# arielgabizon/barretenberg

Hardware: AMD Instinct MI355X
Metric: BN254 G1 MSM points/sec at n=2^20 (Fr NTT elems/sec in 'ntt') (higher is better)
Workload: dtype u32x9 (256-bit Montgomery, 29-bit limbs)

## Files before the change

### barretenberg_amd/csrc/msm.hip

```cpp
#include <hip/hip_runtime.h>

#include <algorithm>
#include <mutex>
#include <stdint.h>
#include <stdio.h>
#include <stdlib.h>
#include <string.h>
#include <vector>

#include "bbgpu_internal.h"
#include "g1.hpp"
#include "g1_quad.hpp"
#include "host_g1.hpp"

namespace bbgpu {

using Fr = FrP;
#define FRONT_PRIO() __builtin_amdgcn_s_setprio(2)
constexpr int TAIL_PRIO = 3;
constexpr int SCALAR_BITS = 254;
constexpr int MSM_MAX_C = 16;
constexpr int MSM_THREADS = 256;

__device__ __forceinline__ void ld8(const uint32_t* p, uint32_t (&w)[8])
{
    const uint4* q = reinterpret_cast<const uint4*>(p);
    uint4 a = q[0], b = q[1];
    w[0] = a.x; w[1] = a.y; w[2] = a.z; w[3] = a.w;
    w[4] = b.x; w[5] = b.y; w[6] = b.z; w[7] = b.w;
}
__device__ __forceinline__ void ld16(const uint32_t* p, uint32_t (&w)[16])
{
    const uint4* q = reinterpret_cast<const uint4*>(p);
#pragma unroll
    for (int i = 0; i < 4; i++) {
        uint4 a = q[i];
        w[4 * i] = a.x; w[4 * i + 1] = a.y; w[4 * i + 2] = a.z; w[4 * i + 3] = a.w;
    }
}
__device__ __forceinline__ void st32(uint32_t* p, const uint32_t (&w)[32])
{
    uint4* q = reinterpret_cast<uint4*>(p);
#pragma unroll
    for (int i = 0; i < 8; i++) q[i] = make_uint4(w[4 * i], w[4 * i + 1], w[4 * i + 2], w[4 * i + 3]);
}
__device__ __forceinline__ void ld32(const uint32_t* p, uint32_t (&w)[32])
{
    const uint4* q = reinterpret_cast<const uint4*>(p);
#pragma unroll
    for (int i = 0; i < 8; i++) {
        uint4 a = q[i];
        w[4 * i] = a.x; w[4 * i + 1] = a.y; w[4 * i + 2] = a.z; w[4 * i + 3] = a.w;
    }
}

struct WinLayout {
    uint16_t off[66];
};
static WinLayout make_layout(int c, bool balanced)
{
    WinLayout LO{};
    const int W = msm_num_windows(c);
    if (!balanced) {
        for (int w = 0; w <= W; w++) LO.off[w] = (uint16_t)(c * w);
        return LO;
    }
    const int base = SCALAR_BITS / W, rem = SCALAR_BITS - base * W;
    int bit = 0;
    for (int w = 0; w < W; w++) {
        LO.off[w] = (uint16_t)bit;
        bit += base + (w < rem ? 1 : 0);
    }
    LO.off[W] = (uint16_t)bit;
    return LO;
}
__global__ void srs_convert_kernel(const uint32_t* __restrict__ table, uint32_t* __restrict__ srs, uint32_t n, uint32_t stride_words)
{
    const uint32_t i = blockIdx.x * blockDim.x + threadIdx.x;
    if (i >= n) return;
    uint32_t w[16];
    ld16(table + (size_t)i * stride_words, w);
    AffineV<2> a;
    load_affine_m256(a, w);
    uint32_t o[16];
    store_affine_m261(o, a.x, a.y);
    uint4* q = reinterpret_cast<uint4*>(srs + (size_t)i * 16);
#pragma unroll
    for (int k = 0; k < 4; k++) q[k] = make_uint4(o[4 * k], o[4 * k + 1], o[4 * k + 2], o[4 * k + 3]);
}

__global__ void srs_export_kernel(const uint32_t* __restrict__ srs, uint32_t* __restrict__ table, uint32_t n)
{
    const uint32_t i = blockIdx.x * blockDim.x + threadIdx.x;
    if (i >= n) return;
    uint32_t w[16];
    ld16(srs + (size_t)i * 16, w);
// ... 78 lines not shown
    return pow_u256<Fq>(a, e);
}
__global__ void srs_gen_points_kernel(const uint32_t* __restrict__ tab, Limbs9 x261, uint32_t* __restrict__ srs, uint32_t n, uint32_t first)
{
    const uint32_t i = blockIdx.x * blockDim.x + threadIdx.x;
    if (i >= n) return;
    Fe<Fr, 1, 2> s = fe_one<Fr>(), b = fe_from<Fr>(x261.d);
    for (uint32_t e = first + i; e; e >>= 1) {
        if (e & 1) s = mul(s, b);
        b = sqr(b);
    }
    uint32_t k[8];
    {
        FeT<Fr> one_raw = fe_zero<Fr>();
        one_raw.d[0] = 1;
        to_canonical(mul(s, one_raw), k);
    }
    Xyzz acc;
    set_infinity(acc);
    for (uint32_t w = 0; w < 32; w++) {
        const uint32_t d = (k[w >> 2] >> ((w & 3) * 8)) & 0xff;
        if (d) {
            uint32_t pw[32];
            ld32(tab + ((size_t)w * 256 + d) * 32, pw);
            Xyzz q;
            load_xyzz(q, pw);
            Xyzz t;
            add(t, acc, q);
            acc = t;
        }
    }
    auto inv = fq_inverse(mul(acc.zz, acc.zzz));
    auto izz = mul(inv, acc.zzz), izzz = mul(inv, acc.zz);
    uint32_t o[16];
    store_affine_m261(o, mul(acc.x, izz), mul(acc.y, izzz));
    uint4* q = reinterpret_cast<uint4*>(srs + (size_t)i * 16);
#pragma unroll
    for (int t = 0; t < 4; t++) q[t] = make_uint4(o[4 * t], o[4 * t + 1], o[4 * t + 2], o[4 * t + 3]);
}

struct ScalarSets {
    const uint32_t* p[MSM_MAX_JOBS];
};
template <class DT> struct DigitTraits { static constexpr bool wide = false; };
template <> struct DigitTraits<uint16_t> { static constexpr bool wide = true; };
template <class DT> __device__ __forceinline__ int load_digit(const DT* __restrict__ dg, const unsigned long long* __restrict__ sg, uint32_t i)
{
    if constexpr (DigitTraits<DT>::wide) {
        const int u = dg[i];
        return ((sg[i >> 6] >> (i & 63u)) & 1ull) ? -u - 1 : u;
    } else {
        return dg[i];
    }
}
template <class DT> __device__ __forceinline__ void load_digits8(const DT* __restrict__ dg, const unsigned long long* __restrict__ sg, uint32_t i8, int (&d)[8])
{
    const uint4 q = *reinterpret_cast<const uint4*>(dg + i8);
    const uint32_t w[4] = { q.x, q.y, q.z, q.w };
    if constexpr (DigitTraits<DT>::wide) {
        const uint32_t sb = reinterpret_cast<const uint8_t*>(sg)[i8 >> 3];
#pragma unroll
        for (int k = 0; k < 8; k++) {
            const int u = (int)((w[k >> 1] >> (16 * (k & 1))) & 0xffffu);
            d[k] = ((sb >> k) & 1u) ? -u - 1 : u;
        }
    } else {
#pragma unroll
        for (int k = 0; k < 8; k++) d[k] = (int)(int16_t)(w[k >> 1] >> (16 * (k & 1)));
    }
}
template <class DT> __global__ void __launch_bounds__(MSM_THREADS) msm_digits_kernel(ScalarSets sets, DT* __restrict__ digits_all, unsigned long long* __restrict__ signs_all,
                                                               uint32_t n, WinLayout LO, uint32_t num_windows, uint32_t wb, uint32_t we)
{
    FRONT_PRIO();
    const uint32_t i = blockIdx.x * blockDim.x + threadIdx.x;
    if (i >= n) return;
    const uint32_t* __restrict__ scalars = sets.p[blockIdx.y];
    DT* __restrict__ digits = digits_all + (size_t)blockIdx.y * num_windows * n;
    const uint32_t s64 = (n + 63) >> 6;
    unsigned long long* __restrict__ signs = signs_all + (size_t)blockIdx.y * num_windows * s64;
    uint32_t w[8], k[9];
    ld8(scalars + (size_t)i * 8, w);
    to_canonical(exact_limbs(mul(unpack<Fr>(w), fe_from<Fr>(Fr::M256_TO_PLAIN))), w);
#pragma unroll
    for (int j = 0; j < 8; j++) k[j] = w[j];
    k[8] = 0;
    uint32_t carry = 0;
    for (uint32_t win = 0; win < we; win++) {
        const uint32_t bit = LO.off[win], sz = LO.off[win + 1] - bit, j = bit >> 5, s = bit & 31;
        const uint32_t half = 1u << (sz - 1), mask = (1u << sz) - 1;
        uint32_t v = 0;
        if (j < 8) {
            v = k[j] >> s;
            if (s + sz > 32) v |= k[j + 1] << (32 - s);
        }
        v = (v & mask) + carry;
        carry = (win + 1 < num_windows && v >= half) ? 1u : 0u;
        const int32_t d = (int32_t)v - (int32_t)(carry << sz);
        if (win >= wb) {
            if constexpr (DigitTraits<DT>::wide) {
                const unsigned long long neg = __ballot(d < 0);
                digits[(size_t)win * n + i] = (DT)(d < 0 ? -d - 1 : d);
                if ((threadIdx.x & 63u) == 0) signs[(size_t)win * s64 + (i >> 6)] = neg;
            } else {
                digits[(size_t)win * n + i] = (DT)d;
            }
        }
    }
}

constexpr int SORT_THREADS = 1024;
constexpr uint32_t SORT_MAX_LB = 7;
constexpr uint32_t SORTB_MAX_PARTS = 8;
constexpr uint32_t SORTB_SPLIT_MIN = 1u << 16;

__device__ __forceinline__ bool wave_keys_heavy(bool valid, uint32_t key)
{
    const uint64_t vm = __ballot(valid);
    if (!vm) return false;
    const uint32_t k0 = __builtin_amdgcn_readlane(key, __ffsll((unsigned long long)vm) - 1);
    return 4 * __popcll(__ballot(valid && key == k0)) >= __popcll(vm);
}
__device__ __forceinline__ uint32_t lds_inc_dedup(uint32_t* ctr, uint32_t key, bool heavy)
{
    if (!heavy) return atomicAdd(&ctr[key], 1u);
    const uint32_t lane = __lane_id();
    uint64_t todo = __ballot(1);
    uint32_t res = 0;
    for (int it = 0; it < 4 && todo; it++) {
        const int leader = __ffsll((unsigned long long)todo) - 1;
        const uint32_t kk = __builtin_amdgcn_readlane(key, leader);
        const uint64_t m = __ballot(key == kk) & todo;
        uint32_t base = 0;
        if ((int)lane == leader) base = atomicAdd(&ctr[kk], (uint32_t)__popcll(m));
        base = __builtin_amdgcn_readlane(base, leader);
        if ((m >> lane) & 1ull) res = base + (uint32_t)__popcll(m & ((1ull << lane) - 1ull));
        todo &= ~m;
    }
    if ((todo >> lane) & 1ull) res = atomicAdd(&ctr[key], 1u);
    return res;
}

template <class DT> __global__ void __launch_bounds__(SORT_THREADS) __attribute__((amdgpu_num_vgpr(32))) sortA_hist_kernel(const DT* __restrict__ digits, const unsigned long long* __restrict__ signs, uint32_t* __restrict__ histA, uint32_t n,
                                                                uint32_t bins, uint32_t lb, uint32_t slices, uint32_t slice_len, uint32_t win0,
                                                                uint32_t wpg, uint32_t first_i0, uint32_t last_i1, uint32_t blo, uint32_t bcnt)
{
    FRONT_PRIO();
    __shared__ uint32_t lh[SORT_THREADS];
    const uint32_t s = blockIdx.x, wl = blockIdx.y;
    lh[threadIdx.x] = 0;
    __syncthreads();
    const uint32_t lo = s * slice_len, hi = min(n, lo + slice_len);
    const uint32_t s64 = (n + 63) >> 6;
    if ((n & 7u) == 0) {
        const uint32_t lo8 = lo & ~7u, bpw = lo < hi ? (((hi + 7u) & ~7u) - lo8) >> 3 : 0u;
        for (uint32_t u = threadIdx.x; u < wpg * bpw; u += SORT_THREADS) {
            const uint32_t k = u / bpw, i8 = lo8 + (u - k * bpw) * 8;
            const uint32_t klo = (k == 0) ? max(lo, first_i0) : lo, khi = (k + 1 == wpg) ? min(hi, last_i1) : hi;
            int d[8];
            load_digits8<DT>(digits + (size_t)(win0 + wl * wpg + k) * n, signs + (size_t)(win0 + wl * wpg + k) * s64, i8, d);
            const bool heavy = wave_keys_heavy(d[0] != 0, (uint32_t)((d[0] < 0 ? -d[0] : d[0]) - 1) >> lb);
#pragma unroll
            for (int j = 0; j < 8; j++)
                if (d[j] && i8 + j >= klo && i8 + j < khi) {
                    const uint32_t b = (uint32_t)((d[j] < 0 ? -d[j] : d[j]) - 1);
                    if (b - blo < bcnt) (void)lds_inc_dedup(lh, b >> lb, heavy);
                }
        }
    } else {
        for (uint32_t k = 0; k < wpg; k++) {
            const DT* dg = digits + (size_t)(win0 + wl * wpg + k) * n;
            const unsigned long long* sg = signs + (size_t)(win0 + wl * wpg + k) * s64;
            const uint32_t klo = (k == 0) ? max(lo, first_i0) : lo, khi = (k + 1 == wpg) ? min(hi, last_i1) : hi;
            for (uint32_t i = klo + threadIdx.x; i < khi; i += SORT_THREADS) {
                const int d = load_digit<DT>(dg, sg, i);
                if (d) {
                    const uint32_t b = (uint32_t)((d < 0 ? -d : d) - 1);
                    if (b - blo < bcnt) atomicAdd(&lh[b >> lb], 1u);
                }
            }
        }
// ... 342 lines not shown
            if (base + k * THREADS + t < end) buf[toff[(v[k] >> 24) & 0x7f] + rk[k]] = v[k];
        __syncthreads();
        const uint32_t tile_n = min(TILE, end - base);
        for (uint32_t x = t; x < tile_n; x += THREADS) {
            const uint32_t w = buf[x];
            sorted[dlt[(w >> 24) & 0x7f] + x] = w & 0x80ffffffu;
        }
    }
}

__device__ __forceinline__ void store_raw(uint32_t* dst, const Xyzz& p)
{
#if defined(__HIP_DEVICE_COMPILE__)
    uint32_t v[4 * NL];
#pragma unroll
    for (int i = 0; i < NL; i++) { v[i] = p.x.d[i]; v[NL + i] = p.y.d[i]; v[2 * NL + i] = p.zz.d[i]; v[3 * NL + i] = p.zzz.d[i]; }
#pragma unroll
    for (int i = 0; i < 4 * NL; i += 2)
        asm volatile("global_store_dwordx2 %0, %1, off offset:%2" :: "v"(dst), "v"(((unsigned long long)v[i + 1] << 32) | v[i]), "n"(4 * i) : "memory");
#else
#pragma unroll
    for (int i = 0; i < NL; i++) {
        dst[i] = p.x.d[i];
        dst[NL + i] = p.y.d[i];
        dst[2 * NL + i] = p.zz.d[i];
        dst[3 * NL + i] = p.zzz.d[i];
    }
#endif
}
__device__ __forceinline__ void load_raw(Xyzz& p, const uint32_t* src)
{
#pragma unroll
    for (int i = 0; i < NL; i++) {
        p.x.d[i] = src[i];
        p.y.d[i] = src[NL + i];
        p.zz.d[i] = src[2 * NL + i];
        p.zzz.d[i] = src[3 * NL + i];
    }
}
typedef uint32_t u32x4 __attribute__((ext_vector_type(4)));
struct RowRegs { u32x4 q0, q1, q2, q3; };
__device__ __forceinline__ void row_request(RowRegs& r, const uint32_t* p)
{
#if defined(__HIP_DEVICE_COMPILE__)
    asm volatile("global_load_dwordx4 %0, %4, off\n\t"
                 "global_load_dwordx4 %1, %4, off offset:16\n\t"
                 "global_load_dwordx4 %2, %4, off offset:32\n\t"
                 "global_load_dwordx4 %3, %4, off offset:48"
                 : "=&v"(r.q0), "=&v"(r.q1), "=&v"(r.q2), "=&v"(r.q3) : "v"(p) : "memory");
#else
    const u32x4* q = reinterpret_cast<const u32x4*>(p);
    r.q0 = q[0]; r.q1 = q[1]; r.q2 = q[2]; r.q3 = q[3];
#endif
}
__device__ __forceinline__ void row_land(RowRegs& r, uint32_t (&w)[16])
{
#if defined(__HIP_DEVICE_COMPILE__)
    __builtin_amdgcn_s_waitcnt(0x0f70);
    asm volatile("" : "+v"(r.q0), "+v"(r.q1), "+v"(r.q2), "+v"(r.q3));
#endif
#pragma unroll
    for (int i = 0; i < 4; i++) { w[i] = r.q0[i]; w[4 + i] = r.q1[i]; w[8 + i] = r.q2[i]; w[12 + i] = r.q3[i]; }
}
__device__ __forceinline__ void value_landed(uint32_t& v)
{
#if defined(__HIP_DEVICE_COMPILE__)
    asm volatile("" : "+v"(v));
#endif
}
__device__ __forceinline__ void operand_done(Fe<Fq, 1, 1>& x, Fe<Fq, 1, 2>& y)
{
#if defined(__HIP_DEVICE_COMPILE__)
    asm volatile("" : "+v"(x.d[0]), "+v"(x.d[1]), "+v"(x.d[2]), "+v"(x.d[3]), "+v"(x.d[4]), "+v"(x.d[5]), "+v"(x.d[6]), "+v"(x.d[7]), "+v"(x.d[8]));
    asm volatile("" : "+v"(y.d[0]), "+v"(y.d[1]), "+v"(y.d[2]), "+v"(y.d[3]), "+v"(y.d[4]), "+v"(y.d[5]), "+v"(y.d[6]), "+v"(y.d[7]), "+v"(y.d[8]));
#endif
}
constexpr int RAW_WORDS = 4 * NL;
constexpr uint32_t HEAVY_WGS = 256;
constexpr uint32_t HEAVY_IDS = 1 + HEAVY_WGS;
static_assert(MSM_THREADS == (int)HEAVY_WGS, "heavy-bucket queue header is cleared / combined by one lane per K4h workgroup");

__global__ void __launch_bounds__(MSM_THREADS) msm_accumulate_kernel(const uint32_t* __restrict__ srs, const uint32_t* __restrict__ sorted,
                                                                   const uint32_t* __restrict__ gstart, uint32_t* __restrict__ partials,
                                                                   uint32_t total_buckets, uint32_t ch, uint32_t prio, uint32_t* __restrict__ heavy_counter)
{
    if (heavy_counter && blockIdx.x == 0) {
        heavy_counter[threadIdx.x] = 0;
        if (threadIdx.x == 0) heavy_counter[MSM_THREADS] = 0;
    }
    if (prio == 1) __builtin_amdgcn_s_setprio(1);
    else if (prio == 2) __builtin_amdgcn_s_setprio(2);
    const uint32_t t = blockIdx.x * blockDim.x + threadIdx.x;
    const uint32_t M = gstart[total_buckets];
    const uint32_t p0 = t * ch;
    if (p0 >= M) return;
    const uint32_t p1 = min(M, p0 + ch);
    uint32_t lo = 0, hi = total_buckets;
    while (hi - lo > 1) {
        const uint32_t mid = (lo + hi) >> 1;
        if (gstart[mid] <= p0) lo = mid; else hi = mid;
    }
    uint32_t b = lo;
    uint32_t next_end = gstart[b + 1];
    Xyzz acc;
    set_infinity(acc);
    uint32_t after_next = gstart[min(b + 2, total_buckets + 1)];
    bool acc_inf = true;
    uint32_t v = sorted[p0];
    uint32_t vn = sorted[p0 + 1 < p1 ? p0 + 1 : p0];
    RowRegs row;
    uint32_t w[16];
    row_request(row, srs + (size_t)(v & 0x7fffffffu) * 16);
    Fe<Fq, 1, 1> px;
    Fe<Fq, 1, 2> py;
    row_land(row, w);
    load_affine_m261_signed(px, py, w, (v >> 31) != 0);
    operand_done(px, py);
    row_request(row, srs + (size_t)(vn & 0x7fffffffu) * 16);
    uint32_t e = p0;
    uint32_t trips = ch;
    do {
        const uint32_t vnn = sorted[min(e + 2, p1 - 1)];
        const bool start = (e == next_end) || acc_inf;
        if (start) {
            if (e == next_end) {
                store_raw(partials + (size_t)(b + t) * RAW_WORDS, acc);
                b++;
                next_end = after_next;
                if (next_end <= e) {
                    if (e >= M) {
                        b = total_buckets;
                    } else {
                        uint32_t l2 = b, h2 = total_buckets;
                        while (h2 - l2 > 1) {
                            const uint32_t mid = (l2 + h2) >> 1;
                            if (gstart[mid] <= e) l2 = mid; else h2 = mid;
                        }
                        b = l2;
                    }
                    next_end = gstart[b + 1];
                    value_landed(next_end);
                }
                after_next = gstart[min(b + 2, total_buckets + 1)];
            }
            acc.x = px;
            acc.y = py;
            acc.zz = fe_one<Fq>();
            acc.zzz = fe_one<Fq>();
            acc_inf = false;
        }
        asm volatile("" ::: "memory");
        if (!start) madd_ip(acc, acc_inf, px, py);
        row_land(row, w);
        load_affine_m261_signed(px, py, w, (vn >> 31) != 0);
        operand_done(px, py);
        row_request(row, srs + (size_t)(vnn & 0x7fffffffu) * 16);
        vn = vnn;
        e++;
    } while (--trips != 0);
    store_raw(partials + (size_t)(b + t) * RAW_WORDS, acc);
}

__device__ __forceinline__ Xyzz shfl_down_xyzz(const Xyzz& p, uint32_t off)
{
    Xyzz r;
#pragma unroll
    for (int i = 0; i < NL; i++) {
        r.x.d[i] = __shfl_down(p.x.d[i], off);
        r.y.d[i] = __shfl_down(p.y.d[i], off);
        r.zz.d[i] = __shfl_down(p.zz.d[i], off);
        r.zzz.d[i] = __shfl_down(p.zzz.d[i], off);
    }
    return r;
}
#define TAIL_OCC __attribute__((amdgpu_waves_per_eu(4, 4)))
constexpr int FOLD_T = 256;
constexpr int FOLD_LDS_WORDS = (FOLD_T / 2) * RAW_WORDS;
__device__ __forceinline__ void wg_tree_sum(Xyzz& acc, uint32_t* sh, uint32_t T, uint32_t t)
{
    constexpr uint32_t STRIDE = FOLD_T / 2;
    for (uint32_t half = T >> 1; half >= 1; half >>= 1) {
        if (t >= half && t < 2 * half) {
#pragma unroll
            for (int i = 0; i < NL; i++) {
                sh[(0 * NL + i) * STRIDE + t - half] = acc.x.d[i];
                sh[(1 * NL + i) * STRIDE + t - half] = acc.y.d[i];
                sh[(2 * NL + i) * STRIDE + t - half] = acc.zz.d[i];
                sh[(3 * NL + i) * STRIDE + t - half] = acc.zzz.d[i];
            }
        }
        __syncthreads();
        if (t < half) {
            Xyzz q, r;
#pragma unroll
            for (int i = 0; i < NL; i++) {
                q.x.d[i] = sh[(0 * NL + i) * STRIDE + t];
                q.y.d[i] = sh[(1 * NL + i) * STRIDE + t];
                q.zz.d[i] = sh[(2 * NL + i) * STRIDE + t];
                q.zzz.d[i] = sh[(3 * NL + i) * STRIDE + t];
            }
            add(r, acc, q);
            acc = r;
        }
        __syncthreads();
    }
}
__global__ void __launch_bounds__(MSM_THREADS) TAIL_OCC msm_merge_kernel(const uint32_t* __restrict__ gstart, const uint32_t* __restrict__ partials,
                                                              uint32_t* __restrict__ buckets, uint32_t* __restrict__ heavy, uint32_t bucket_begin, uint32_t total_buckets,
                                                              uint32_t ch, uint32_t MERGE_LIGHT, uint32_t logG)
{
    __builtin_amdgcn_s_setprio(TAIL_PRIO);
    const uint32_t t = blockIdx.x * blockDim.x + threadIdx.x;
    const uint32_t G = 1u << logG, b = bucket_begin + (t >> logG), j = t & (G - 1);
    if (b >= total_buckets) return;
    const uint32_t s = gstart[b], e = gstart[b + 1];
    Xyzz acc;
    set_infinity(acc);
    if (e > s) {
        const uint32_t t0 = s / ch, t1 = (e - 1) / ch;
        if (t1 - t0 >= MERGE_LIGHT) {
            if (j == 0) heavy[HEAVY_IDS + atomicAdd(&heavy[0], 1u)] = b;
            return;
        }
        for (uint32_t k = t0 + j; k <= t1; k += G) {
            Xyzz q, r;
            load_raw(q, partials + (size_t)(b + k) * RAW_WORDS);
            add(r, acc, q);
            acc = r;
        }
    }
    for (uint32_t off = G >> 1; off >= 1; off >>= 1) {
        const Xyzz o = shfl_down_xyzz(acc, off);
        if (j < off) {
            Xyzz r;
            add(r, acc, o);
            acc = r;
        }
    }
    if (j == 0) {
        uint32_t o[32];
        store_xyzz(o, acc);
        st32(buckets + (size_t)b * 32, o);
    }
}
__global__ void __launch_bounds__(MSM_THREADS) TAIL_OCC msm_merge_heavy_kernel(const uint32_t* __restrict__ gstart, const uint32_t* __restrict__ partials,
                                                                    uint32_t* __restrict__ buckets, uint32_t* __restrict__ heavy, uint32_t ch, uint32_t* __restrict__ hpart)
{
    __builtin_amdgcn_s_setprio(TAIL_PRIO);
    __shared__ uint32_t sh[FOLD_LDS_WORDS];
    __shared__ uint32_t last_flag;
    const uint32_t count = heavy[0];
    const uint32_t K = count ? gridDim.x / count : 0;
    if (K < 2) {
        for (uint32_t item = blockIdx.x; item < count; item += gridDim.x) {
            const uint32_t b = heavy[HEAVY_IDS + item];
            const uint32_t s = gstart[b], e = gstart[b + 1];
            const uint32_t t0 = s / ch, t1 = (e - 1) / ch;
            Xyzz acc;
            set_infinity(acc);
            for (uint32_t t = t0 + threadIdx.x; t <= t1; t += MSM_THREADS) {
                Xyzz q, r;
                load_raw(q, partials + (size_t)(b + t) * RAW_WORDS);
                add(r, acc, q);
                acc = r;
            }
            __syncthreads();
            wg_tree_sum(acc, sh, MSM_THREADS, threadIdx.x);
            if (threadIdx.x == 0) {
                uint32_t o[32];
                store_xyzz(o, acc);
                st32(buckets + (size_t)b * 32, o);
            }
        }
        return;
    }
    const uint32_t item = blockIdx.x / K, sub = blockIdx.x - item * K;
    if (item >= count) return;
    const uint32_t b = heavy[HEAVY_IDS + item];
    const uint32_t s = gstart[b], e = gstart[b + 1];
    const uint32_t t0 = s / ch, t1 = (e - 1) / ch, total = t1 - t0 + 1;
    const uint32_t lo = t0 + (uint32_t)(((uint64_t)total * sub) / K), hi = t0 + (uint32_t)(((uint64_t)total * (sub + 1)) / K);
    Xyzz acc;
    set_infinity(acc);
    for (uint32_t t = lo + threadIdx.x; t < hi; t += MSM_THREADS) {
        Xyzz q, r;
        load_raw(q, partials + (size_t)(b + t) * RAW_WORDS);
        add(r, acc, q);
        acc = r;
    }
    wg_tree_sum(acc, sh, MSM_THREADS, threadIdx.x);
    if (threadIdx.x == 0) {
        store_raw(hpart + (size_t)blockIdx.x * RAW_WORDS, acc);
        __threadfence();
        last_flag = (atomicAdd(&heavy[1 + item], 1u) == K - 1) ? 1u : 0u;
    }
    __syncthreads();
    if (!last_flag) return;
    __threadfence();
    set_infinity(acc);
    if (threadIdx.x < K) load_raw(acc, hpart + (size_t)(item * K + threadIdx.x) * RAW_WORDS);
    __syncthreads();
    wg_tree_sum(acc, sh, MSM_THREADS, threadIdx.x);
    if (threadIdx.x == 0) {
        uint32_t o[32];
        store_xyzz(o, acc);
        st32(buckets + (size_t)b * 32, o);
    }
}

__device__ __forceinline__ uint32_t insert_one_bit(uint32_t m, uint32_t k)
{
    return ((m >> k) << (k + 1)) | (1u << k) | (m & ((1u << k) - 1));
}
constexpr int QFOLD_T = 256;
__device__ __forceinline__ FqN quad_load(const uint32_t* point32, uint32_t l)
{
    const uint4* q = reinterpret_cast<const uint4*>(point32 + 8 * l);
    const uint4 a = q[0], b = q[1];
    const uint32_t w[8] = { a.x, a.y, a.z, a.w, b.x, b.y, b.z, b.w };
    return FqN(unpack<Fq>(w));
}
__device__ __forceinline__ FqN quad_zero()
{
    return FqN(fe_zero<Fq>());
}
template <int T = QFOLD_T> __device__ __forceinline__ FqN block_quad_sum(FqN acc, uint32_t* sh , uint32_t t, uint32_t active = T / 4)
{
    const uint32_t l = t & 3, lane = t & 63, wave = t >> 6, qd = lane >> 2;
    const uint32_t in_wave = active > 16 * wave ? min(16u, active - 16 * wave) : 0u;
    for (uint32_t off = 8; off >= 1; off >>= 1) {
        if (off >= in_wave) continue;
        FqN o;
#pragma unroll
        for (int i = 0; i < NL; i++) o.d[i] = __shfl_down(acc.d[i], off * 4);
        if (qd < off) acc = quad_add(acc, o, l);
    }
    if constexpr (T == 64) return acc;
    constexpr uint32_t NW = T / 64;
    const uint32_t waves = min(NW, (active + 15) / 16);
    if (waves <= 1) return acc;
    if (lane < 4) {
#pragma unroll
        for (int i = 0; i < NL; i++) sh[(wave * 4 + l) * NL + i] = acc.d[i];
    }
    __syncthreads();
    if (wave == 0) {
        acc = quad_zero();
        if (qd < NW) {
#pragma unroll
            for (int i = 0; i < NL; i++) acc.d[i] = sh[(qd * 4 + l) * NL + i];
        }
        for (uint32_t off = NW >> 1; off >= 1; off >>= 1) {
            if (off >= waves) continue;
            FqN o;
#pragma unroll
            for (int i = 0; i < NL; i++) o.d[i] = __shfl_down(acc.d[i], off * 4);
            if (qd < off) acc = quad_add(acc, o, l);
        }
    }
    return acc;
}
__device__ __forceinline__ void quad_store8(uint32_t* dst8, const uint32_t (&w)[8])
{
    uint4* q = reinterpret_cast<uint4*>(dst8);
    q[0] = make_uint4(w[0], w[1], w[2], w[3]);
    q[1] = make_uint4(w[4], w[5], w[6], w[7]);
}

__global__ void __launch_bounds__(MSM_THREADS) TAIL_OCC msm_merge_quad_kernel(const uint32_t* __restrict__ gstart, const uint32_t* __restrict__ partials,
                                                                   uint32_t* __restrict__ buckets, uint32_t* __restrict__ heavy, uint32_t bucket_begin, uint32_t total_buckets,
                                                                   uint32_t ch, uint32_t MERGE_LIGHT, uint32_t logQ)
{
    __builtin_amdgcn_s_setprio(TAIL_PRIO);
    const uint32_t t = blockIdx.x * blockDim.x + threadIdx.x, l = t & 3, quad = t >> 2;
    const uint32_t Q = 1u << logQ, b = bucket_begin + (quad >> logQ), j = quad & (Q - 1);
    if (b >= total_buckets) return;
    const uint32_t s = gstart[b], e = gstart[b + 1];
    FqN acc = quad_zero();
    if (e > s) {
        const uint32_t t0 = s / ch, t1 = (e - 1) / ch;
        if (t1 - t0 >= MERGE_LIGHT) {
            if (j == 0 && l == 0) heavy[HEAVY_IDS + atomicAdd(&heavy[0], 1u)] = b;
            return;
        }
        uint32_t k = t0 + j;
        if (k <= t1) {
            const uint32_t* src = partials + (size_t)(b + k) * RAW_WORDS + NL * l;
#pragma unroll
            for (int i = 0; i < NL; i++) acc.d[i] = src[i];
            FqN q = quad_zero();
            k += Q;
            if (k <= t1) {
                src = partials + (size_t)(b + k) * RAW_WORDS + NL * l;
#pragma unroll
                for (int i = 0; i < NL; i++) q.d[i] = src[i];
            }
            while (k <= t1) {
                FqN qn = quad_zero();
                const uint32_t kn = k + Q;
                if (kn <= t1) {
                    src = partials + (size_t)(b + kn) * RAW_WORDS + NL * l;
#pragma unroll
                    for (int i = 0; i < NL; i++) qn.d[i] = src[i];
                }
                acc = quad_add(acc, q, l);
                q = qn;
                k = kn;
            }
        }
    }
    for (uint32_t off = Q >> 1; off >= 1; off >>= 1) {
        FqN o;
#pragma unroll
        for (int i = 0; i < NL; i++) o.d[i] = __shfl_down(acc.d[i], off * 4);
        if (j < off) acc = quad_add(acc, o, l);
    }
    if (j == 0) {
        uint32_t w[8];
        to_canonical(acc, w);
        quad_store8(buckets + (size_t)b * 32 + 8 * l, w);
    }
}

__global__ void __launch_bounds__(QFOLD_T) TAIL_OCC msm_rowcol_quad_kernel(const uint32_t* __restrict__ buckets, uint32_t* __restrict__ R, uint32_t* __restrict__ Cc,
                                                                  uint32_t H, uint32_t L, uint32_t* __restrict__ zero_out, uint32_t zero_words, uint32_t r0, uint32_t rows)
{
    __builtin_amdgcn_s_setprio(TAIL_PRIO);
    __shared__ uint32_t sh[(QFOLD_T / 64) * 4 * NL];
    const uint32_t g = blockIdx.y, t = threadIdx.x, nb = H * L, l = t & 3, quad = t >> 2;
    if (zero_out) {
        const uint32_t gid = (g * gridDim.x + blockIdx.x) * blockDim.x + t, all = gridDim.y * gridDim.x * blockDim.x;
        for (uint32_t i = gid; i < zero_words; i += all) zero_out[i] = 0;
    }
    const bool row = blockIdx.x < rows;
    const uint32_t idx = row ? r0 + blockIdx.x : blockIdx.x - rows, count = row ? L : rows;
    FqN acc = quad_zero();
    bool first = true;
    for (uint32_t e = quad; e < count; e += QFOLD_T / 4) {
        const size_t b = row ? (size_t)idx * L + e : (size_t)(r0 + e) * L + idx;
        const FqN v = quad_load(buckets + ((size_t)g * nb + b) * 32, l);
        acc = first ? v : quad_add(acc, v, l);
        first = false;
    }
    acc = block_quad_sum(acc, sh, t, min(count, (uint32_t)QFOLD_T / 4));
    if (t < 4) {
        uint32_t w[8];
        to_canonical(acc, w);
        quad_store8((row ? R + ((size_t)g * H + idx) * 32 : Cc + ((size_t)g * L + idx) * 32) + 8 * l, w);
    }
}
constexpr uint32_t ROWCOL_SEG = 4;
__global__ void __launch_bounds__(MSM_THREADS) TAIL_OCC msm_rowcol_seg_kernel(const uint32_t* __restrict__ buckets, uint32_t* __restrict__ segs, uint32_t H, uint32_t L,
                                                                                                                uint32_t* __restrict__ zero_out, uint32_t zero_words)
{
    __builtin_amdgcn_s_setprio(TAIL_PRIO);
    const uint32_t g = blockIdx.y, t = blockIdx.x * blockDim.x + threadIdx.x, nb = H * L;
    if (zero_out) {
        const uint32_t gid = g * gridDim.x * blockDim.x + t, all = gridDim.y * gridDim.x * blockDim.x;
        for (uint32_t i = gid; i < zero_words; i += all) zero_out[i] = 0;
// ... 333 lines not shown
    if (PC.hout_group + G > MSM_HOUT_GROUPS) {
        set_error("MSM in %d pieces of %u bucket sets: the result array holds %u", S.npieces + 1, G, MSM_HOUT_GROUPS);
        return BBGPU_ERR_SIZE;
    }
    int rc = ws.ensure(MsmWorkspace::bytes_needed(n, c, (int)nw, (int)G));
    if (rc) return rc;
    if (!ws.h_out) HIPCHK(hipHostMalloc((void**)&ws.h_out, (size_t)MSM_HOUT_GROUPS * 64 * 128));
    if (!S.done) HIPCHK(hipEventCreateWithFlags(&S.done, hipEventDisableTiming));

    const MsmCarve LY = carve(P, n, nw, G);
    if (LY.end > ws.cap) {
        set_error("internal: MSM workspace of %zu bytes, layout needs %zu (n=%zu c=%d nw=%u)", ws.cap, LY.end, n, c, nw);
        return BBGPU_ERR_STATE;
    }
    uint8_t* const p = ws.base;
    void* digits = (void*)(p + LY.digits);
    unsigned long long* signs = (unsigned long long*)(p + LY.signs);
    uint32_t* histA = (uint32_t*)(p + LY.histA);
    uint32_t* histB = (uint32_t*)(p + LY.histB);
    uint32_t* binstart = (uint32_t*)(p + LY.binstart);
    uint32_t* bintot = (uint32_t*)(p + LY.bintot);
    uint32_t* tmp_entries = (uint32_t*)(p + LY.tmp_entries);
    uint32_t* gstart = (uint32_t*)(p + LY.gstart);
    uint32_t* totals = (uint32_t*)(p + LY.totals);
    uint32_t* bases = totals + nw;
    uint32_t* heavy = (uint32_t*)(p + LY.heavy);
    uint32_t* sorted = (uint32_t*)(p + LY.sorted);
    uint32_t* partials = (uint32_t*)(p + LY.partials);
    uint32_t* buckets = (uint32_t*)(p + LY.buckets);
    uint32_t* scratch = (uint32_t*)(p + LY.arena);
    if ((uint64_t)G * slices * sort_bins > (uint64_t)nw * P.slices * 1024 || sort_bins > 1024 ||
        (size_t)G * ((size_t)(1u << P.hbits) + (size_t)(1u << P.lbits)) + 64 > arena_points(P, G)) {
        set_error("internal: MSM launch shape exceeds the workspace layout");
        return BBGPU_ERR_STATE;
    }

    hipEvent_t* ev = S.ev;
    const bool tm = want_timing == 1, tm_acc = want_timing != 0;
    S.timed_light = want_timing == 2;
    if (tm_acc) {
        if (!S.ev[0])
            for (int i = 0; i < 8; i++) HIPCHK(hipEventCreate(&S.ev[i]));
        if (tm) HIPCHK(hipEventRecord(ev[0], st));
        S.timed = true;
    }

    if (bshare) {
        HIPCHK(hipMemsetAsync(scratch, 0, (size_t)G * BH * 128, st));
    }
    ScalarSets sets{};
    for (int j = 0; j < jobs; j++) sets.p[j] = (const uint32_t*)d_scalars_v[j];
    const bool wide = c > 16;
    if (wide) msm_digits_kernel<uint16_t><<<dim3((P.n + MSM_THREADS - 1) / MSM_THREADS, jobs), MSM_THREADS, 0, st>>>(sets, (uint16_t*)digits, signs, P.n, make_layout(c, table), P.W, (uint32_t)wb, (uint32_t)we);
    else msm_digits_kernel<int16_t><<<dim3((P.n + MSM_THREADS - 1) / MSM_THREADS, jobs), MSM_THREADS, 0, st>>>(sets, (int16_t*)digits, signs, P.n, make_layout(c, table), P.W, (uint32_t)wb, (uint32_t)we);
    if (tm) HIPCHK(hipEventRecord(ev[1], st));
    if (wide) sortA_hist_kernel<uint16_t><<<dim3(slices, G), SORT_THREADS, 0, st>>>((const uint16_t*)digits, signs, histA, P.n, sort_bins, sort_lb, slices, slice_len, (uint32_t)wb, wpg, row_i0, row_i1, blo, bcnt);
    else sortA_hist_kernel<int16_t><<<dim3(slices, G), SORT_THREADS, 0, st>>>((const int16_t*)digits, signs, histA, P.n, sort_bins, sort_lb, slices, slice_len, (uint32_t)wb, wpg, row_i0, row_i1, blo, bcnt);
    sortA_colscan_kernel<<<dim3((sort_bins + SORT_THREADS / 64 - 1) / (SORT_THREADS / 64), G), SORT_THREADS, 0, st>>>(histA, bintot, sort_bins, slices);
    sortA_scan_kernel<<<G, SORT_THREADS, 0, st>>>(bintot, binstart, totals, sort_bins, G == 1 ? bases : nullptr, gstart + (size_t)G * P.nb);
    if (G > 1) sort_bases_kernel<<<1, 64, 0, st>>>(totals, bases, gstart + (size_t)G * P.nb, G);
    if ((P.n & 7u) == 0) {
        if (wide) sortA_scatter_staged_kernel<uint16_t><<<dim3(slices, G), SORT_THREADS, 0, st>>>((const uint16_t*)digits, signs, histA, binstart, bases, tmp_entries, P.n, sort_bins, sort_lb, slices,
                                                                                  slice_len, (uint32_t)wb, wpg, idx_stride, P.W, row_i0, row_i1, blo, bcnt);
        else sortA_scatter_staged_kernel<int16_t><<<dim3(slices, G), SORT_THREADS, 0, st>>>((const int16_t*)digits, signs, histA, binstart, bases, tmp_entries, P.n, sort_bins, sort_lb, slices,
                                                                            slice_len, (uint32_t)wb, wpg, idx_stride, P.W, row_i0, row_i1, blo, bcnt);
    } else if (wide) sortA_scatter_kernel<uint16_t><<<dim3(slices, G), SORT_THREADS, 0, st>>>((const uint16_t*)digits, signs, histA, binstart, bases, tmp_entries, P.n, sort_bins, sort_lb, slices,
                                                                   slice_len, (uint32_t)wb, wpg, idx_stride, P.W, row_i0, row_i1, blo, bcnt);
    else sortA_scatter_kernel<int16_t><<<dim3(slices, G), SORT_THREADS, 0, st>>>((const int16_t*)digits, signs, histA, binstart, bases, tmp_entries, P.n, sort_bins, sort_lb, slices,
                                                                   slice_len, (uint32_t)wb, wpg, idx_stride, P.W, row_i0, row_i1, blo, bcnt);
    if (table) {
        uint32_t parts = ((uint64_t)n * nw1 >= ((uint64_t)1 << 21) && G <= MSM_MAX_JOBS) ? SORTB_MAX_PARTS : 1u;
        if ((size_t)G * sort_bins * parts * 128 * 4 > LY.histB_bytes) parts = 1;
        if (parts > 1) sortB_count_kernel<SORT_THREADS><<<dim3(sort_bins, G, parts), SORT_THREADS, 0, st>>>(tmp_entries, binstart, bases, histB, sort_bins, parts);
        sortB_staged_kernel<SORT_THREADS><<<dim3(sort_bins, G, parts), SORT_THREADS, 0, st>>>(tmp_entries, binstart, bases, sorted, gstart, sort_bins, sort_lb, P.nb, histB, parts);
    } else sortB_staged_kernel<256><<<dim3(sort_bins, G), 256, 0, st>>>(tmp_entries, binstart, bases, sorted, gstart, sort_bins, sort_lb, P.nb, nullptr, 1u);
    if (tm_acc) HIPCHK(hipEventRecord(ev[2], st));
    const uint32_t total_buckets = G * P.nb;
    const uint64_t m_expected = bshare ? std::max<uint64_t>(1, (uint64_t)n * nw * bcnt / P.nb) : (uint64_t)n * nw;
    const uint32_t merge_buckets = bshare ? bcnt : total_buckets;
    const bool tp = hint && jobs == 1;
    constexpr uint32_t TP_MIN_CHUNK = 20;
    uint32_t ch = bshare ? chunk_len_m(m_expected) : chunk_len(n, nw);
    ch = std::max(ch, min_chunk((uint64_t)n * nw));
    if (tp && ch < TP_MIN_CHUNK)
        ch = std::max(ch, std::min<uint32_t>(TP_MIN_CHUNK, (uint32_t)(m_expected / (acc_capacity_lanes() / ACC_WG_PER_CU))));
    const uint32_t avg_partials = (uint32_t)(m_expected / ((uint64_t)merge_buckets * ch)) + 1;
    uint32_t logG = 0;
    while ((1u << logG) < avg_partials && logG < 6 && ((uint64_t)merge_buckets << (logG + 1)) <= ((uint64_t)1 << 16)) logG++;
    const uint32_t merge_light = std::max(6u, 8u << logG);
    const uint32_t max_chunks = (uint32_t)(((uint64_t)n * nw + ch - 1) / ch);
    msm_accumulate_kernel<<<(max_chunks + MSM_THREADS - 1) / MSM_THREADS, MSM_THREADS, 0, st>>>(points, sorted, gstart, partials, total_buckets, ch, 0, heavy);
    if (tm_acc) {
        HIPCHK(hipEventRecord(ev[3], st));
        if (int rc = acc_ring_record(S, st)) return rc;
    } else {
        S.acc_seq = 0;
    }
    if ((uint64_t)n * nw <= ((uint64_t)1 << 21)) {
        uint32_t logQ = 0;
        while ((2u << logQ) < avg_partials && logQ < 4 && ((uint64_t)merge_buckets << (logQ + 3)) <= ((uint64_t)1 << 17)) logQ++;
        msm_merge_quad_kernel<<<(uint32_t)((((uint64_t)merge_buckets << (logQ + 2)) + MSM_THREADS - 1) / MSM_THREADS), MSM_THREADS, 0, st>>>(gstart, partials, buckets, heavy, blo, blo + merge_buckets, ch,
                                                                                                                                  std::max(32u, 8u << logQ), logQ);
    } else msm_merge_kernel<<<(uint32_t)((((uint64_t)merge_buckets << logG) + MSM_THREADS - 1) / MSM_THREADS), MSM_THREADS, 0, st>>>(gstart, partials, buckets, heavy,
                                                                                                                     blo, blo + merge_buckets, ch, merge_light, logG);
    msm_merge_heavy_kernel<<<HEAVY_WGS, MSM_THREADS, 0, st>>>(gstart, partials, buckets, heavy, ch, heavy + (((size_t)G * P.nb + HEAVY_IDS + 63) & ~(size_t)63));
    if (tm) HIPCHK(hipEventRecord(ev[4], st));

    const uint32_t H = 1u << P.hbits, L = 1u << P.lbits;
    {
        uint32_t* Rr = scratch;
        uint32_t* Cc = scratch + (size_t)G * H * 32;
        uint32_t* const dest = (uint32_t*)ws.h_out + (size_t)PC.hout_group * 64 * 32;
        const uint32_t zero_words = G * 64 * 32;
        if (!bshare && rowcol_two_step(P) && (tp || jobs > 1)) {
            uint32_t* segs = (uint32_t*)(p + LY.segs);
            const uint32_t seg_lanes = 2 * (H * L / ROWCOL_SEG);
            msm_rowcol_seg_kernel<<<dim3((seg_lanes + MSM_THREADS - 1) / MSM_THREADS, G), MSM_THREADS, 0, st>>>(buckets, segs, H, L, dest, zero_words);
            msm_segsum_quad_kernel<<<dim3(H + L, G), 64, 0, st>>>(segs, Rr, Cc, H, L);
        } else msm_rowcol_quad_kernel<<<dim3((bshare ? brow1 - brow0 : H) + L, G), QFOLD_T, 0, st>>>(buckets, Rr, Cc, H, L, dest, zero_words, bshare ? brow0 : 0u,
                                                                                                  bshare ? brow1 - brow0 : H);
        if (tm) HIPCHK(hipEventRecord(ev[5], st));
        msm_final_quad_kernel<<<dim3(1 + P.hbits + P.lbits, G), QFOLD_T, 0, st>>>(Rr, Cc, dest, P.hbits, P.lbits);
        if (tm) HIPCHK(hipEventRecord(ev[6], st));
    }
    HIPCHK(hipEventRecord(S.done, st));
    HIPCHK(launch_check());
    S.npieces++;
    S.pending = true;
    return BBGPU_OK;
}

static host::Xyzz group_sum(const MsmSlot& S, const MsmPiece& PC, uint32_t w)
{
    auto pt = [&](uint32_t slot) {
        host::Xyzz q;
        memcpy(&q, (const uint8_t*)S.ws.h_out + ((size_t)(PC.hout_group + w) * 64 + slot) * 128, 128);
        return q;
    };
    host::Xyzz rs = host::g1_infinity();
    for (int k = (int)PC.hbits - 1; k >= 0; --k) rs = host::g1_add(host::g1_dbl(rs), pt(1 + k));
    for (uint32_t k = 0; k < PC.lbits; k++) rs = host::g1_dbl(rs);
    host::Xyzz cs = host::g1_infinity();
    for (int k = (int)PC.lbits - 1; k >= 0; --k) cs = host::g1_add(host::g1_dbl(cs), pt(32 + k));
    return host::g1_add(host::g1_add(rs, cs), pt(0));
}
static int finish_timing(MsmSlot& S, MsmTiming* timing)
{
    if (S.timed && timing) {
        float ms;
        timing->count = 0;
        if (S.timed_light) {
            for (int i = 0; i < 7; i++) timing->ms[timing->count++] = 0.0f;
            HIPCHK(hipEventElapsedTime(&ms, S.ev[2], S.ev[3]));
            timing->ms[3] = ms;
        } else {
            HIPCHK(hipEventElapsedTime(&ms, S.ev[0], S.ev[6]));
            timing->ms[timing->count++] = ms;
            for (int i = 0; i < 6; i++) {
                HIPCHK(hipEventElapsedTime(&ms, S.ev[i], S.ev[i + 1]));
                timing->ms[timing->count++] = ms;
            }
        }
        float exec = timing->ms[3];
        const AccRing* R = S.acc_ring;
        if (R && S.acc_seq > 1 && R->seq - (S.acc_seq - 1) < (uint64_t)ACC_RING &&
            hipEventElapsedTime(&ms, R->end[(S.acc_seq - 1) % ACC_RING], R->end[S.acc_seq % ACC_RING]) == hipSuccess && ms > 0.0f && ms < exec)
            exec = ms;
        (void)hipGetLastError();
        timing->ms[timing->count++] = exec;
    }
    return BBGPU_OK;
}
static int msm_finish(MsmSlot& S, host::Xyzz* result, MsmTiming* timing)
{
    *result = host::g1_infinity();
    if (!S.pending) return BBGPU_ERR_STATE;
    if (S.jobs > 1) return BBGPU_ERR_STATE;
    S.pending = false;
    bool waited = false;
    host::Xyzz total = host::g1_infinity();
    for (int pi = 0; pi < S.npieces; pi++) {
        const MsmPiece& PC = S.piece[pi];
        if (PC.trivial) continue;
        if (!waited) HIPCHK(hipEventSynchronize(S.done));
        waited = true;
        host::Xyzz acc = host::g1_infinity();
        for (int w = (int)PC.nw - 1; w >= 0; --w) {
            for (uint32_t k = 0; k < PC.c; k++) acc = host::g1_dbl(acc);
// ... 116 lines not shown
```

Baseline: 958.3 million.

## Negate large scalars to shrink digits and size chunks from actual bucket count

The digit kernel now conditionally negates each scalar (k -> r - k when k exceeds r/2) and flips the sign of every signed digit. This keeps the top window small and makes fewer points land in high buckets. Chunk length for the accumulate and merge kernels is now computed on the device from the real sorted-list length M via a ChunkRule (capped at the host chunk, floored at a minimum), instead of a fixed host value based on the expected count. This should spread the work evenly across the launched lanes when M falls short of the estimate, at the cost of an extra gstart read and a division in each kernel.

```diff
diff --git a/barretenberg_amd/csrc/msm.hip b/barretenberg_amd/csrc/msm.hip
--- a/barretenberg_amd/csrc/msm.hip
+++ b/barretenberg_amd/csrc/msm.hip
@@ -12,6 +12,7 @@
 #include "g1.hpp"
 #include "g1_quad.hpp"
 #include "host_g1.hpp"
+#include "msm_chunk.hpp"
 
 namespace bbgpu {
 
@@ -256,8 +257,19 @@
     uint32_t w[8], k[9];
     ld8(scalars + (size_t)i * 8, w);
     to_canonical(exact_limbs(mul(unpack<Fr>(w), fe_from<Fr>(Fr::M256_TO_PLAIN))), w);
-#pragma unroll
-    for (int j = 0; j < 8; j++) k[j] = w[j];
+    constexpr uint32_t R32[8] = { 0xf0000001u, 0x43e1f593u, 0x79b97091u, 0x2833e848u, 0x8181585du, 0xb85045b6u, 0xe131a029u, 0x30644e72u };
+    constexpr uint32_t H32[8] = { 0xf8000001u, 0xa1f0fac9u, 0x3cdcb848u, 0x9419f424u, 0x40c0ac2eu, 0xdc2822dbu, 0x7098d014u, 0x18322739u };
+    uint32_t borrow = 0;
+#pragma unroll
+    for (int j = 0; j < 8; j++) (void)__builtin_subc(w[j], H32[j], borrow, &borrow);
+    const uint32_t negk = borrow ^ 1u, nm = 0u - negk;
+    {
+        uint32_t c = negk;
+#pragma unroll
+        for (int j = 0; j < 8; j++) {
+            k[j] = __builtin_addc(w[j] ^ nm, R32[j] & nm, c, &c);
+        }
+    }
     k[8] = 0;
     uint32_t carry = 0;
     for (uint32_t win = 0; win < we; win++) {
@@ -269,8 +281,8 @@
             if (s + sz > 32) v |= k[j + 1] << (32 - s);
         }
         v = (v & mask) + carry;
-        carry = (win + 1 < num_windows && v >= half) ? 1u : 0u;
-        const int32_t d = (int32_t)v - (int32_t)(carry << sz);
+        carry = (win + 1 < num_windows && v >= half + negk) ? 1u : 0u;
+        const int32_t d = (int32_t)((v - (carry << sz)) ^ nm) + (int32_t)negk;
         if (win >= wb) {
             if constexpr (DigitTraits<DT>::wide) {
                 const unsigned long long neg = __ballot(d < 0);
@@ -779,7 +791,7 @@
 
 __global__ void __launch_bounds__(MSM_THREADS) msm_accumulate_kernel(const uint32_t* __restrict__ srs, const uint32_t* __restrict__ sorted,
                                                                    const uint32_t* __restrict__ gstart, uint32_t* __restrict__ partials,
-                                                                   uint32_t total_buckets, uint32_t ch, uint32_t prio, uint32_t* __restrict__ heavy_counter)
+                                                                   uint32_t total_buckets, ChunkRule rule, uint32_t prio, uint32_t* __restrict__ heavy_counter)
 {
     if (heavy_counter && blockIdx.x == 0) {
         heavy_counter[threadIdx.x] = 0;
@@ -789,6 +801,7 @@
     else if (prio == 2) __builtin_amdgcn_s_setprio(2);
     const uint32_t t = blockIdx.x * blockDim.x + threadIdx.x;
     const uint32_t M = gstart[total_buckets];
+    const uint32_t ch = __builtin_amdgcn_readfirstlane(chunk_len_dev(M, rule));
     const uint32_t p0 = t * ch;
     if (p0 >= M) return;
     const uint32_t p1 = min(M, p0 + ch);
@@ -904,12 +917,13 @@
 }
 __global__ void __launch_bounds__(MSM_THREADS) TAIL_OCC msm_merge_kernel(const uint32_t* __restrict__ gstart, const uint32_t* __restrict__ partials,
                                                               uint32_t* __restrict__ buckets, uint32_t* __restrict__ heavy, uint32_t bucket_begin, uint32_t total_buckets,
-                                                              uint32_t ch, uint32_t MERGE_LIGHT, uint32_t logG)
+                                                              ChunkRule rule, uint32_t list_end, uint32_t MERGE_LIGHT, uint32_t logG)
 {
     __builtin_amdgcn_s_setprio(TAIL_PRIO);
     const uint32_t t = blockIdx.x * blockDim.x + threadIdx.x;
     const uint32_t G = 1u << logG, b = bucket_begin + (t >> logG), j = t & (G - 1);
     if (b >= total_buckets) return;
+    const uint32_t ch = chunk_len_dev(gstart[list_end], rule);
     const uint32_t s = gstart[b], e = gstart[b + 1];
     Xyzz acc;
     set_infinity(acc);
@@ -941,12 +955,13 @@
     }
 }
 __global__ void __launch_bounds__(MSM_THREADS) TAIL_OCC msm_merge_heavy_kernel(const uint32_t* __restrict__ gstart, const uint32_t* __restrict__ partials,
-                                                                    uint32_t* __restrict__ buckets, uint32_t* __restrict__ heavy, uint32_t ch, uint32_t* __restrict__ hpart)
+                                                                    uint32_t* __restrict__ buckets, uint32_t* __restrict__ heavy, ChunkRule rule, uint32_t list_end, uint32_t* __restrict__ hpart)
 {
     __builtin_amdgcn_s_setprio(TAIL_PRIO);
     __shared__ uint32_t sh[FOLD_LDS_WORDS];
     __shared__ uint32_t last_flag;
     const uint32_t count = heavy[0];
+    const uint32_t ch = chunk_len_dev(gstart[list_end], rule);
     const uint32_t K = count ? gridDim.x / count : 0;
     if (K < 2) {
         for (uint32_t item = blockIdx.x; item < count; item += gridDim.x) {
@@ -1066,12 +1081,13 @@
 
 __global__ void __launch_bounds__(MSM_THREADS) TAIL_OCC msm_merge_quad_kernel(const uint32_t* __restrict__ gstart, const uint32_t* __restrict__ partials,
                                                                    uint32_t* __restrict__ buckets, uint32_t* __restrict__ heavy, uint32_t bucket_begin, uint32_t total_buckets,
-                                                                   uint32_t ch, uint32_t MERGE_LIGHT, uint32_t logQ)
+                                                                   ChunkRule rule, uint32_t list_end, uint32_t MERGE_LIGHT, uint32_t logQ)
 {
     __builtin_amdgcn_s_setprio(TAIL_PRIO);
     const uint32_t t = blockIdx.x * blockDim.x + threadIdx.x, l = t & 3, quad = t >> 2;
     const uint32_t Q = 1u << logQ, b = bucket_begin + (quad >> logQ), j = quad & (Q - 1);
     if (b >= total_buckets) return;
+    const uint32_t ch = chunk_len_dev(gstart[list_end], rule);
     const uint32_t s = gstart[b], e = gstart[b + 1];
     FqN acc = quad_zero();
     if (e > s) {
@@ -1571,14 +1587,19 @@
     constexpr uint32_t TP_MIN_CHUNK = 20;
     uint32_t ch = bshare ? chunk_len_m(m_expected) : chunk_len(n, nw);
     ch = std::max(ch, min_chunk((uint64_t)n * nw));
-    if (tp && ch < TP_MIN_CHUNK)
-        ch = std::max(ch, std::min<uint32_t>(TP_MIN_CHUNK, (uint32_t)(m_expected / (acc_capacity_lanes() / ACC_WG_PER_CU))));
+    uint32_t ch_floor = min_chunk((uint64_t)n * nw);
+    if (tp && ch < TP_MIN_CHUNK) {
+        const uint32_t tp_min = std::min<uint32_t>(TP_MIN_CHUNK, (uint32_t)(m_expected / (acc_capacity_lanes() / ACC_WG_PER_CU)));
+        ch = std::max(ch, tp_min);
+        ch_floor = std::max(ch_floor, tp_min);
+    }
+    const ChunkRule rule{ ch, ch_floor, (uint32_t)(((m_expected + ch - 1) / ch + MSM_THREADS - 1) / MSM_THREADS * MSM_THREADS) };
     const uint32_t avg_partials = (uint32_t)(m_expected / ((uint64_t)merge_buckets * ch)) + 1;
     uint32_t logG = 0;
     while ((1u << logG) < avg_partials && logG < 6 && ((uint64_t)merge_buckets << (logG + 1)) <= ((uint64_t)1 << 16)) logG++;
     const uint32_t merge_light = std::max(6u, 8u << logG);
     const uint32_t max_chunks = (uint32_t)(((uint64_t)n * nw + ch - 1) / ch);
-    msm_accumulate_kernel<<<(max_chunks + MSM_THREADS - 1) / MSM_THREADS, MSM_THREADS, 0, st>>>(points, sorted, gstart, partials, total_buckets, ch, 0, heavy);
+    msm_accumulate_kernel<<<(max_chunks + MSM_THREADS - 1) / MSM_THREADS, MSM_THREADS, 0, st>>>(points, sorted, gstart, partials, total_buckets, rule, 0, heavy);
     if (tm_acc) {
         HIPCHK(hipEventRecord(ev[3], st));
         if (int rc = acc_ring_record(S, st)) return rc;
@@ -1588,11 +1609,11 @@
     if ((uint64_t)n * nw <= ((uint64_t)1 << 21)) {
         uint32_t logQ = 0;
         while ((2u << logQ) < avg_partials && logQ < 4 && ((uint64_t)merge_buckets << (logQ + 3)) <= ((uint64_t)1 << 17)) logQ++;
-        msm_merge_quad_kernel<<<(uint32_t)((((uint64_t)merge_buckets << (logQ + 2)) + MSM_THREADS - 1) / MSM_THREADS), MSM_THREADS, 0, st>>>(gstart, partials, buckets, heavy, blo, blo + merge_buckets, ch,
-                                                                                                                                  std::max(32u, 8u << logQ), logQ);
+        msm_merge_quad_kernel<<<(uint32_t)((((uint64_t)merge_buckets << (logQ + 2)) + MSM_THREADS - 1) / MSM_THREADS), MSM_THREADS, 0, st>>>(gstart, partials, buckets, heavy, blo, blo + merge_buckets, rule,
+                                                                                                                                  total_buckets, std::max(32u, 8u << logQ), logQ);
     } else msm_merge_kernel<<<(uint32_t)((((uint64_t)merge_buckets << logG) + MSM_THREADS - 1) / MSM_THREADS), MSM_THREADS, 0, st>>>(gstart, partials, buckets, heavy,
-                                                                                                                     blo, blo + merge_buckets, ch, merge_light, logG);
-    msm_merge_heavy_kernel<<<HEAVY_WGS, MSM_THREADS, 0, st>>>(gstart, partials, buckets, heavy, ch, heavy + (((size_t)G * P.nb + HEAVY_IDS + 63) & ~(size_t)63));
+                                                                                                                     blo, blo + merge_buckets, rule, total_buckets, merge_light, logG);
+    msm_merge_heavy_kernel<<<HEAVY_WGS, MSM_THREADS, 0, st>>>(gstart, partials, buckets, heavy, rule, total_buckets, heavy + (((size_t)G * P.nb + HEAVY_IDS + 63) & ~(size_t)63));
     if (tm) HIPCHK(hipEventRecord(ev[4], st));
 
     const uint32_t H = 1u << P.hbits, L = 1u << P.lbits;
diff --git a/barretenberg_amd/csrc/msm_chunk.hpp b/barretenberg_amd/csrc/msm_chunk.hpp
--- /dev/null
+++ b/barretenberg_amd/csrc/msm_chunk.hpp
@@ -0,0 +1,20 @@
+#pragma once
+#include <stdint.h>
+
+#if defined(__HIPCC__)
+#define MSM_CHUNK_HD __host__ __device__ __forceinline__
+#else
+#define MSM_CHUNK_HD inline
+#endif
+
+struct ChunkRule {
+    uint32_t ch;
+    uint32_t floor;
+    uint32_t lanes;
+};
+MSM_CHUNK_HD uint32_t chunk_len_dev(uint32_t M, ChunkRule R)
+{
+    const uint32_t q = M / R.lanes, need = q + (M - q * R.lanes != 0u ? 1u : 0u);
+    const uint32_t lo = need > R.floor ? need : R.floor;
+    return lo < R.ch ? lo : R.ch;
+}
```

Result: slower. 948.6 million (-1.0%).
